# scrasmussen/uoparallel-seismic-project

Hardware: NVIDIA B200
Metric: GRelax/s (higher is better)
Workload: dtype f32

## Files before the change

include/sweeptt.h:

```cpp
#ifndef SWEEPTT_H
#define SWEEPTT_H

#include <stddef.h>
#include <stdint.h>

#ifdef __cplusplus
extern "C" {
#endif

#ifndef SWEEPTT_NO_STRUCTS
struct FS {
  int i, j, k;
  float d;
};

struct START {
  int i, j, k;
};
#endif

enum {
  SWEEPTT_KERNEL_AUTO = 0,
  SWEEPTT_KERNEL_SIMPLE = 1,
  SWEEPTT_KERNEL_TILED = 2
// ... 138 lines not shown
  int struct_size;
  double damp, smooth;
  double atol, btol, conlim;
  int iter_lim;
} sweeptt_lsqr_opts;

typedef struct {
  int struct_size;
  int istop, itn;
  double r1norm, r2norm, anorm, acond, arnorm, xnorm;
} sweeptt_lsqr_info;

int sweeptt_rayset_lsqr(sweeptt_rayset *set, const uint8_t *rows,
                        const double *b,
                        const sweeptt_lsqr_opts *opts,
                        double *x_out,
                        sweeptt_lsqr_info *info,
                        sweeptt_stats *stats);


enum { SWEEPTT_LOC_OK = 0, SWEEPTT_LOC_NO_PICKS = 1, SWEEPTT_LOC_UNREACHED = 2 };

int sweeptt_locate_events(sweeptt_ctx *ctx, int source_begin, int source_count, const float *picks, int nev,
                          struct START *best_out, float *misfit_out, double *origin_out,
                          int32_t *npicks_out, int32_t *status_out, sweeptt_stats *stats);

int sweeptt_misfit_box(sweeptt_ctx *ctx, int source_begin, int source_count, const float *picks ,
                       float *misfit_out, sweeptt_stats *stats);

long long sweeptt_relaxations_per_round(sweeptt_ctx *ctx);
size_t sweeptt_pool_bytes(sweeptt_ctx *ctx);
long long sweeptt_tiles_per_source(sweeptt_ctx *ctx);
int sweeptt_debug_model_stats(sweeptt_ctx *ctx, float *vmin, float *vmax, float *vpos);


int sweeptt_solve_slabs(const float *slowness, int nx, int ny, int nz, const struct FS *fs,
                        int starsize, struct START start, float *tt_out, const sweeptt_opts *opts,
                        sweeptt_stats *stats);

int sweeptt_solve_slabs_vbox(const char *vbox_path, const struct FS *fs, int starsize, struct START start,
                             float *tt_out, const sweeptt_opts *opts, sweeptt_stats *stats);


int sweeptt_vbox_load(const char *path, float **slowness, int origin[3], int dims[3]);
int sweeptt_vbox_dims(const char *path, int dims[3]);
int sweeptt_vbox_store(const char *path, const float *slowness, const int origin[3],
                       const int dims[3]);
int sweeptt_vbox_load_subset(const char *path, const int sub_origin[3], const int sub_dims[3],
                             float **slowness);
int sweeptt_text_load(const char *path, float **slowness, int origin[3], int dims[3]);
int sweeptt_star_load(const char *path, float delta, struct FS **fs, int *starsize);
int sweeptt_starts_load(const char *path, struct START **starts, int *numstart);
int sweeptt_write_output_tt(const char *path, const float *const *tt, int numstart, int nx, int ny,
                            int nz);
void sweeptt_free(void *p);

#ifdef __cplusplus
}
#endif
#endif
```

uoparallel_seismic_project_b200/api.py:

```python
from __future__ import annotations

import ctypes as C
import os
import pathlib
import weakref
from dataclasses import dataclass

import numpy as np

_PKG = pathlib.Path(__file__).resolve().parent
_LIB = None

KERNEL_AUTO, KERNEL_SIMPLE, KERNEL_TILED = 0, 1, 2
LOOP_AUTO, LOOP_BATCHED, LOOP_GRAPH = 0, 1, 2
RAY_OK, RAY_UNREACHED, RAY_NOT_FIXED_POINT, RAY_NO_PREDECESSOR, RAY_STALLED, RAY_TRUNCATED = range(6)
LOC_OK, LOC_NO_PICKS, LOC_UNREACHED = range(3)


class SweepError(RuntimeError):
    pass


class FS(C.Structure):
    _fields_ = [("i", C.c_int), ("j", C.c_int), ("k", C.c_int), ("d", C.c_float)]
# ... 42 lines not shown
    relaxations: int = 0
    solve_ms: float = 0.0
    relax_kernel_ms: float = 0.0
    relax_launches: int = 0
    h2d_ms: float = 0.0
    d2h_ms: float = 0.0
    h2d_bytes: int = 0
    d2h_bytes: int = 0
    units_run: int = 0
    units_changed: int = 0

    @classmethod
    def _from(cls, s: _Stats) -> "SweepStats":
        return cls(**{f: getattr(s, f) for f in cls.__dataclass_fields__})


def lib_path() -> pathlib.Path:
    import os
    if os.environ.get("SWEEPTT_LIB"):
        return pathlib.Path(os.environ["SWEEPTT_LIB"])
    return _PKG / "lib" / "libsweeptt.so"


_EXPORTS = [
    "sweeptt_device_count", "sweeptt_device_info", "sweeptt_last_error", "sweeptt_version",
    "sweeptt_star_fill_distances", "sweeptt_build_pull_star", "sweeptt_debug_column_split", "sweeptt_solve", "sweeptt_release_cache",
    "sweeptt_host_alloc", "sweeptt_host_free",
    "sweeptt_create", "sweeptt_destroy", "sweeptt_set_stream", "sweeptt_set_model", "sweeptt_set_star",
    "sweeptt_set_sources", "sweeptt_run", "sweeptt_step", "sweeptt_reset", "sweeptt_get_tt", "sweeptt_put_tt",
    "sweeptt_count_violations", "sweeptt_trace_rays", "sweeptt_ray_project", "sweeptt_ray_backproject",
    "sweeptt_rayset_freeze", "sweeptt_rayset_destroy", "sweeptt_rayset_bytes", "sweeptt_rayset_table",
    "sweeptt_rayset_paths", "sweeptt_rayset_project", "sweeptt_rayset_backproject", "sweeptt_rayset_lsqr",
    "sweeptt_locate_events",
    "sweeptt_misfit_box", "sweeptt_relaxations_per_round", "sweeptt_pool_bytes", "sweeptt_tiles_per_source", "sweeptt_debug_model_stats", "sweeptt_solve_slabs",
    "sweeptt_solve_slabs_vbox", "sweeptt_vbox_dims",
    "sweeptt_vbox_load", "sweeptt_vbox_store", "sweeptt_vbox_load_subset", "sweeptt_text_load",
    "sweeptt_star_load", "sweeptt_starts_load", "sweeptt_write_output_tt", "sweeptt_free",
]


def load_library() -> C.CDLL:
    global _LIB
    if _LIB is not None:
        return _LIB
    p = lib_path()
    if not p.exists():
        raise SweepError(f"{p} is missing: run `python -c 'import __graft_entry__ as g; g.build()'` "
                         "(the sweep has no CPU fallback)")
    lib = C.CDLL(str(p))
    fp, ip = C.POINTER(C.c_float), C.POINTER(C.c_int)
    lib.sweeptt_last_error.restype = C.c_char_p
    lib.sweeptt_version.restype = C.c_char_p
    lib.sweeptt_device_info.argtypes = [C.c_int, C.c_char_p, C.c_int, ip, ip, C.POINTER(C.c_size_t)]
    lib.sweeptt_star_fill_distances.argtypes = [C.POINTER(FS), C.c_int, C.c_float]
    lib.sweeptt_star_fill_distances.restype = None
    lib.sweeptt_build_pull_star.argtypes = [C.POINTER(FS), C.c_int, C.c_int, C.c_void_p, C.c_void_p, C.c_void_p, C.c_int]
    lib.sweeptt_solve.argtypes = [C.c_void_p, C.c_int, C.c_int, C.c_int, C.POINTER(FS), C.c_int, C.POINTER(START),
                                  C.c_int, C.POINTER(C.c_void_p), C.POINTER(_Opts), C.POINTER(_Stats)]
    lib.sweeptt_release_cache.restype = None
    lib.sweeptt_host_alloc.argtypes = [C.c_size_t]
    lib.sweeptt_host_alloc.restype = C.c_void_p
    lib.sweeptt_host_free.argtypes = [C.c_void_p]
    lib.sweeptt_host_free.restype = None
    lib.sweeptt_create.argtypes = [C.POINTER(_Opts)]
    lib.sweeptt_create.restype = C.c_void_p
    lib.sweeptt_destroy.argtypes = [C.c_void_p]
    lib.sweeptt_destroy.restype = None
# ... 7 lines not shown
    lib.sweeptt_get_tt.argtypes = [C.c_void_p, C.c_int, C.c_void_p]
    lib.sweeptt_put_tt.argtypes = [C.c_void_p, C.c_int, C.c_void_p]
    lib.sweeptt_count_violations.argtypes = [C.c_void_p, C.c_int, C.POINTER(C.c_longlong)]
    lib.sweeptt_trace_rays.argtypes = [C.c_void_p, C.c_int, C.c_int, C.POINTER(START), C.c_int, C.c_int, C.c_void_p,
                                       C.c_void_p, C.c_void_p, C.c_void_p, C.POINTER(_Stats)]
    lib.sweeptt_ray_project.argtypes = [C.c_void_p, C.c_int, C.c_int, C.POINTER(START), C.c_int, C.c_int, C.c_void_p,
                                        C.c_void_p, C.c_void_p, C.c_void_p, C.POINTER(_Stats)]
    lib.sweeptt_ray_backproject.argtypes = [C.c_void_p, C.c_int, C.c_int, C.POINTER(START), C.c_int, C.c_int,
                                            C.c_void_p, C.c_void_p, C.POINTER(C.c_int), C.c_void_p, C.POINTER(_Stats)]
    lib.sweeptt_rayset_freeze.argtypes = [C.c_void_p, C.c_int, C.c_int, C.POINTER(START), C.c_int, C.c_int,
                                          C.POINTER(_Stats)]
    lib.sweeptt_rayset_freeze.restype = C.c_void_p
    lib.sweeptt_rayset_destroy.argtypes = [C.c_void_p]
    lib.sweeptt_rayset_destroy.restype = None
    lib.sweeptt_rayset_bytes.argtypes = [C.c_void_p]
    lib.sweeptt_rayset_bytes.restype = C.c_size_t
    lib.sweeptt_rayset_table.argtypes = [C.c_void_p, C.c_void_p, C.c_void_p, C.c_void_p]
    lib.sweeptt_rayset_paths.argtypes = [C.c_void_p, C.c_void_p, C.c_void_p]
    lib.sweeptt_rayset_project.argtypes = [C.c_void_p, C.c_void_p, C.c_void_p, C.POINTER(_Stats)]
    lib.sweeptt_rayset_backproject.argtypes = [C.c_void_p, C.c_void_p, C.c_void_p, C.POINTER(C.c_int),
                                               C.POINTER(_Stats)]
    lib.sweeptt_rayset_lsqr.argtypes = [C.c_void_p, C.c_void_p, C.c_void_p, C.POINTER(_LsqrOpts), C.c_void_p,
                                        C.POINTER(_LsqrInfo), C.POINTER(_Stats)]
    lib.sweeptt_locate_events.argtypes = [C.c_void_p, C.c_int, C.c_int, C.c_void_p, C.c_int, C.c_void_p, C.c_void_p,
                                          C.c_void_p, C.c_void_p, C.c_void_p, C.POINTER(_Stats)]
    lib.sweeptt_misfit_box.argtypes = [C.c_void_p, C.c_int, C.c_int, C.c_void_p, C.c_void_p, C.POINTER(_Stats)]
    lib.sweeptt_relaxations_per_round.argtypes = [C.c_void_p]
    lib.sweeptt_relaxations_per_round.restype = C.c_longlong
    lib.sweeptt_pool_bytes.argtypes = [C.c_void_p]
    lib.sweeptt_pool_bytes.restype = C.c_size_t
    lib.sweeptt_tiles_per_source.argtypes = [C.c_void_p]
    lib.sweeptt_tiles_per_source.restype = C.c_longlong
    lib.sweeptt_debug_model_stats.argtypes = [C.c_void_p, C.c_void_p, C.c_void_p, C.c_void_p]
    lib.sweeptt_solve_slabs.argtypes = [C.c_void_p, C.c_int, C.c_int, C.c_int, C.POINTER(FS), C.c_int, START,
                                        C.c_void_p, C.POINTER(_Opts), C.POINTER(_Stats)]
    lib.sweeptt_solve_slabs_vbox.argtypes = [C.c_char_p, C.POINTER(FS), C.c_int, START, C.c_void_p, C.POINTER(_Opts),
                                             C.POINTER(_Stats)]
    lib.sweeptt_vbox_dims.argtypes = [C.c_char_p, ip]
    lib.sweeptt_vbox_load.argtypes = [C.c_char_p, C.POINTER(fp), ip, ip]
    lib.sweeptt_vbox_store.argtypes = [C.c_char_p, C.c_void_p, ip, ip]
    lib.sweeptt_vbox_load_subset.argtypes = [C.c_char_p, ip, ip, C.POINTER(fp)]
    lib.sweeptt_text_load.argtypes = [C.c_char_p, C.POINTER(fp), ip, ip]
    lib.sweeptt_star_load.argtypes = [C.c_char_p, C.c_float, C.POINTER(C.POINTER(FS)), ip]
    lib.sweeptt_starts_load.argtypes = [C.c_char_p, C.POINTER(C.POINTER(START)), ip]
    lib.sweeptt_write_output_tt.argtypes = [C.c_char_p, C.POINTER(C.c_void_p), C.c_int, C.c_int, C.c_int, C.c_int]
    lib.sweeptt_free.argtypes = [C.c_void_p]
    lib.sweeptt_free.restype = None
    _LIB = lib
    return lib


def _check(ok, what: str):
    if not ok:
        raise SweepError(f"{what}: {load_library().sweeptt_last_error().decode()}")


def device_count() -> int:
    return load_library().sweeptt_device_count()


def make_star(offsets, delta: float = 10.0):
    off = np.asarray(offsets, dtype=np.int32).reshape(-1, 3)
    arr = (FS * len(off))()
    for l, (a, b, c) in enumerate(off):
        arr[l].i, arr[l].j, arr[l].k = int(a), int(b), int(c)
    load_library().sweeptt_star_fill_distances(arr, len(off), C.c_float(delta))
# ... 376 lines not shown
                                               status.ctypes.data, C.byref(s)), "sweeptt_locate_events")
        return Locations(node, misfit, origin, npicks, status, SweepStats._from(s))

    def misfit_box(self, picks, sources=None) -> np.ndarray:
        begin, count = self._source_range(sources, "misfit_box")
        p = np.ascontiguousarray(picks, dtype=np.float32)
        if p.shape != (count,):
            raise SweepError(f"misfit_box: picks of shape {p.shape}, expected ({count},)")
        if self.dims is None:
            raise SweepError("misfit_box: the context needs a model first")
        out = np.empty(self.dims, np.float32)
        s = _Stats()
        _check(self._lib.sweeptt_misfit_box(self._h, begin, count, p.ctypes.data, out.ctypes.data, C.byref(s)),
               "sweeptt_misfit_box")
        return out

    @property
    def relaxations_per_round(self) -> int:
        return self._lib.sweeptt_relaxations_per_round(self._h)

    @property
    def tiles_per_source(self) -> int:
        return self._lib.sweeptt_tiles_per_source(self._h)

    @property
    def pool_bytes(self) -> int:
        return self._lib.sweeptt_pool_bytes(self._h)

    def model_stats(self):
        out = np.zeros(3, np.float32)
        _check(self._lib.sweeptt_debug_model_stats(self._h, out[0:].ctypes.data, out[1:].ctypes.data,
                                                   out[2:].ctypes.data), "sweeptt_debug_model_stats")
        return tuple(out)


class RaySet:

    def __init__(self, ctx: SweepContext, handle, shape, dims, stats: SweepStats):
        self._lib = ctx._lib
        self._ctx = ctx
        self._h = handle
        self.shape = shape
        self.dims = dims
        self.stats = stats
        self.length = np.empty(shape, np.int32)
        self.status = np.empty(shape, np.int32)
        self.tt = np.empty(shape, np.float32)
        _check(self._lib.sweeptt_rayset_table(self._h, self.length.ctypes.data, self.status.ctypes.data,
                                              self.tt.ctypes.data), "sweeptt_rayset_table")

    def _handle(self):
        if not self._h:
            raise SweepError("ray set is closed")
        return self._h

    def close(self):
        if getattr(self, "_h", None):
            self._lib.sweeptt_rayset_destroy(self._h)
            self._h = None

    __del__ = close

    def __enter__(self):
        return self

    def __exit__(self, *a):
# ... 210 lines not shown
```

uoparallel_seismic_project_b200/csrc/device_types.h:

```cpp
#pragma once
#include <cstdint>

namespace sweeptt {

#ifndef SWEEPTT_TX
#define SWEEPTT_TX 8
#endif
constexpr int TX = SWEEPTT_TX, TY = 8, TZ = 8, KZ = 8;
static_assert(TX == 4 || TX == 8, "a tile is one or two 4x8x8 units");
constexpr int UNITS = TX / 4;
constexpr int ZHALO = 8;
constexpr int SZD = TZ + 2 * ZHALO + 4;
constexpr int WIN = KZ + 2 * ZHALO;
#ifndef SWEEPTT_NW
#define SWEEPTT_NW 16
#endif
constexpr int MAX_WARPS = SWEEPTT_NW;
constexpr int XREACH = (7 + TX - 1) / TX;
constexpr int NMARK = (2 * XREACH + 1) * 9;

constexpr int AX = 7, AY = 7, AZ = ZHALO;

struct BoxGeom {
  int nx, ny, nz;
  int perm[3];
  long long dstride[3];
  int px, py, pz;
  int ntx, nty, ntz;
  long long sx;
  long long vol;
};

struct SolveState {
  int round;
  int last_changed_round;
  int parity;
  unsigned count[2];
  unsigned cursor;
  unsigned ticket;
  unsigned long long tile_visits;
  unsigned long long pulls;
  unsigned long long units_run;
  unsigned long long units_changed;
  int max_rounds;
  unsigned kmin_bits;
  unsigned ticket2;
  unsigned kmin_pub;
  unsigned gen;
  unsigned builder;
  unsigned done;
  unsigned inflight;
  unsigned long long gslot[4];
};

struct ColumnDev {
  int soff;
  unsigned kmask;
  int hd_begin;
  unsigned gmask;
};

struct ExtraDev {
  int i, j, k;
  int soff;
  float hd;
  int guarded;
  int pad0, pad1;
};

struct StarDev {
  int i, j, k;
  float hd;
  int guarded;
};

struct RayPull {
  short i, j, k;
  unsigned short rank;
  int off;
  float hd;
};
constexpr unsigned RAY_GUARD_BIT = 0x8000u;
constexpr int RAY_MAX_PULLS = 1 << 15;

constexpr int MAX_PARTS = 16;
// ... 9 lines not shown
```

uoparallel_seismic_project_b200/csrc/kernels.cu:

```cuda
#include "kernels.h"

#include "../../include/sweeptt.h"

#include <cuda_runtime.h>
#include <math_constants.h>

#include <algorithm>
#include <cstdint>
#include <limits>

#ifdef SWEEPTT_DEBUG_BOUNDS
#include <cstdio>
#define DBG_BOUNDS(cond)                                                                                        \
  do {                                                                                                          \
    if (!(cond)) {                                                                                              \
      printf("sweeptt bounds check failed: %s (kernels.cu:%d, block %d, thread %d)\n", #cond, __LINE__, (int)blockIdx.x, \
             (int)(threadIdx.y * blockDim.x + threadIdx.x));                                                    \
      __trap();                                                                                                 \
    }                                                                                                           \
  } while (0)
#else
#define DBG_BOUNDS(cond) do { } while (0)
#endif

// ... 353 lines not shown
    const unsigned thr = all ? 0x7f7fffffu : __float_as_uint(kmin + a.bucket);
    const float scale = a.bin_scale;
#pragma unroll 8
    for (unsigned i = tid; i < total; i += NCT) {
      const unsigned k = cache[i];
      if (k != 0x7f800000u && k <= thr) {
        const int b = min(GEN_BINS - 1, (int)((__uint_as_float(k) - kmin) * scale));
        atomicAdd(&s_bin[b + 1], 1u);
      }
    }
    __syncthreads();
    if (tid == 0)
      for (int b = 0; b < GEN_BINS; ++b) s_bin[b + 1] += s_bin[b];
    __syncthreads();
    const unsigned cnt = s_bin[GEN_BINS];
    __syncthreads();
#pragma unroll 8
    for (unsigned i = tid; i < total; i += NCT) {
      const unsigned k = cache[i];
      if (k != 0x7f800000u && k <= thr) {
        const int b = min(GEN_BINS - 1, (int)((__uint_as_float(k) - kmin) * scale));
        wl[atomicAdd(&s_bin[b], 1u)] = i;
        a.key[i] = 0x7f800000u;
        a.busy[i] = 1u;
      }
    }
    __threadfence();
    __syncthreads();
    if (tid == 0) {
      if (cnt != 0) {
        atomicAdd(&S->inflight, cnt);
        atomicExch(&S->gslot[g_new & 3u], (unsigned long long)cnt << 32);
        S->round += 1;
        __threadfence();
        st_volatile_u32(&S->gen, g_new);
        s_stop = 1u;
      } else if (early) {
        st_volatile_u32(&S->builder, g_new - 1u);
        s_stop = 1u;
      } else if (s_inflight == 0u) {
        st_volatile_u32(&S->done, 1u);
        s_stop = 1u;
      } else if (spins > (1u << 22)) {
        st_volatile_u32(&S->done, 2u);
        s_stop = 1u;
      } else {
        __nanosleep(200);
      }
    }
    __syncthreads();
    if (s_stop) break;
  }
}

template <int RXY, typename STAR, int NW, bool PERSIST>
__global__ void __block_size__((32, NW, 1))
relax_tiled(const __grid_constant__ CUtensorMap tm_slow, const __grid_constant__ CUtensorMap tm_tt,
            const __grid_constant__ RelaxArgs a) {
  using D = TileDims<RXY>;
  constexpr int NCT = 32 * NW;
  constexpr int FEED_TID = 32 * (NW / 2 - 1), FIN_WARP = NW - 1;
  extern __shared__ __align__(1024) unsigned char smem_raw[];
  float* ring = reinterpret_cast<float*>(smem_raw + ((128u - (smem_u32(smem_raw) & 127u)) & 127u));
  unsigned* s_acc = reinterpret_cast<unsigned*>(ring + 4 * D::BOX_STRIDE);
  __shared__ __align__(8) uint64_t full[2];
  __shared__ int s_tile[2];
  __shared__ unsigned s_gen;
  __shared__ int s_role;
  __shared__ unsigned s_tmin;
  __shared__ unsigned s_tmax;

  const int lane = threadIdx.x;
  const int wq = threadIdx.y;
  const int tid = wq * 32 + lane;
  if (tid == 0) {
    mbar_init(&full[0], 1); mbar_init(&full[1], 1);
    fence_mbar_init();
    s_tmin = 0x7f800000u;
    s_tmax = 0u;
    s_gen = 0u;
  }
  for (int i = tid; i < D::ACC_WORDS; i += NCT) s_acc[i] = 0x7f800000u;
  __syncthreads();

  SolveState* S = a.st;
  const int par = S->parity;
  const unsigned cnt = S->count[par];
  const unsigned* wl = a.worklist + (size_t)par * a.cap;
  const int round = S->round;
  const int ntiles = a.g.ntx * a.g.nty * a.g.ntz;

  auto stage_tile = [&](int q, int tile) {
    s_tile[q] = tile;
    if (tile < 0) {
      mbar_arrive(&full[q]);
      return;
    }
    if constexpr (PERSIST) fence_proxy_async_global();
    const int s = tile / ntiles;
    int tp = tile - s * ntiles;
    const int tz = tp % a.g.ntz; tp /= a.g.ntz;
    const int ty = tp % a.g.nty;
    const int tx = tp / a.g.nty;
    float* sv = ring + q * 2 * D::BOX_STRIDE;
    DBG_BOUNDS(tile >= 0 && s >= 0 && s < a.nsrc && tx >= 0 && tx < a.g.ntx);
    DBG_BOUNDS(tz * TZ + AZ - ZHALO >= 0 && tz * TZ + AZ - ZHALO + SZD <= a.g.pz);
    DBG_BOUNDS(ty * TY + AY - RXY >= 0 && ty * TY + AY - RXY + D::SYD <= a.g.py);
    DBG_BOUNDS(tx * TX + AX - RXY >= 0 && tx * TX + AX - RXY + D::SXD <= a.g.px);
    DBG_BOUNDS(a.slow_pb == 0 || (a.tx_owner[tx] == a.part && a.tx_slow0[tx] >= 0));
    mbar_expect_tx(&full[q], 2u * sizeof(float) * D::BOX_FLOATS);
    int cx = tx * TX + AX - RXY;
    if (a.slow_pb) cx = a.tx_slow0[tx] + (AX - RXY);
    tma_load_3d(sv, &tm_slow, &full[q], tz * TZ + AZ - ZHALO, ty * TY + AY - RXY, cx);
// ... 32 lines not shown
      const int dx = m / 9 - XREACH, dy = (m / 3) % 3 - 1, dz = m % 3 - 1;
      const int ux = wtx + dx, uy = wty + dy, uz = wtz + dz;
      const bool self = (dx == 0 && dy == 0 && dz == 0);
      bool reach = (abs(dx) - 1) * TX < RXY;
      if (self && !wself) reach = false;
      if (reach && ux >= 0 && ux < a.g.ntx && uy >= 0 && uy < a.g.nty && uz >= 0 && uz < a.g.ntz) {
        const size_t u = (size_t)ws * ntiles + ((size_t)ux * a.g.nty + uy) * a.g.ntz + uz;
        unsigned* keyp = a.key;
        const unsigned* tmaxp = a.tmax;
        if constexpr (!PERSIST) {
          if (a.nparts > 1) {
            const int o = a.tx_owner[ux];
            if ((which == 1 && o != a.part) || (which == 2 && o == a.part)) continue;
            keyp = a.part_key[o];
            tmaxp = a.part_tmax[o];
          }
        }
        bool useful = true;
        if (tmaxp != nullptr && !self)
          useful = __float_as_uint(__fadd_rn(__uint_as_float(wtmin), a.dmin)) < __ldcg(&tmaxp[u]);
        if (useful) atomicMin(&keyp[u], wtmin);
      }
    }
  };
  for (uint32_t it = 0;; ++it) {
    const int q = it & 1;
    mbar_wait(&full[q], (it >> 1) & 1);
    const int tile = s_tile[q];
    if (tile == TILE_NONE) break;
    if constexpr (PERSIST) {
      if (tile == TILE_NEXT_GEN || tile == TILE_BUILD) {
        const bool early = tile == TILE_BUILD;
        __syncthreads();
        for (;;) {
          if (tid == 0) {
            const unsigned g = s_gen;
            int role = 0;
            if (ld_volatile_u32(&S->done)) role = 0;
            else if (ld_volatile_u32(&S->gen) != g) role = 0;
            else if (atomicCAS(&S->builder, g, g + 1u) == g) role = 2;
            else role = early ? 0 : 1;
            s_role = role;
          }
          __syncthreads();
          const int role = s_role;
          __syncthreads();
          if (role == 2) {
          const size_t nkeys = (size_t)a.nsrc * ntiles;
          build_generation<NCT>(a, s_gen + 1u,
                                nkeys <= (size_t)4 * D::BOX_STRIDE ? reinterpret_cast<unsigned*>(ring) : a.keysnap, early);
            fence_proxy_async_all();
            __syncthreads();
            break;
          }
          if (role == 0) break;
          if (tid == 0) {
            unsigned spins = 0;
            while (ld_volatile_u32(&S->gen) == s_gen && !ld_volatile_u32(&S->done) &&
                   ld_volatile_u32(&S->builder) != s_gen) {
              __nanosleep(100);
              if (++spins > (1u << 24)) { st_volatile_u32(&S->done, 2u); break; }
            }
          }
          __syncthreads();
        }
        if (tid == 0) stage_tile(q ^ 1, pop_now());
        continue;
      }
    }
    unsigned pop_i = 0, pop_g = 0, pop_c = 0;
    unsigned long long pop_w = 0;
    int next_tile = TILE_NONE;
    const bool build_now = build_next;
    build_next = false;
    if (tid == FEED_TID) {
      if constexpr (PERSIST) pop_g = s_gen;
      else pop_i = atomicAdd(&S->cursor, 1u);
    }
    const int s = tile / ntiles;
    int tp = tile - s * ntiles;
    const int tz = tp % a.g.ntz; tp /= a.g.ntz;
    const int ty = tp % a.g.nty;
    const int tx = tp / a.g.nty;
    const int x0 = tx * TX, y0 = ty * TY, z0 = tz * TZ;
    const float* sv = ring + q * 2 * D::BOX_STRIDE;
    float* st = ring + q * 2 * D::BOX_STRIDE + D::BOX_STRIDE;

    const int nlive = (UNITS == 2 && x0 + 4 < a.g.nx) ? 2 : 1;
    const int P = NW / nlive;
    const int unit = wq / P, part = wq - unit * P;
    const int xc = tx == 0 ? 1 : (tx == a.g.ntx - 1 ? 2 : 0);
    int f0 = ((xc * 6 + ((PERSIST || a.nparts > 1) ? 3 : 0) + (nlive == 1 ? 0 : 1 + unit)) * MAX_PATTERNS) * MAX_WARPS + part;
#ifndef SWEEPTT_NO_PIN
    asm volatile("" : "+r"(f0));
#endif
    const bool owner = part == 0;
    const int x = (unit << 2) | (lane >> 3);
    const int b0 = ((x + RXY) * D::SYD + (y + RXY)) * SZD;
// ... 1233 lines not shown
    default: return cudaErrorInvalidValue;
  }
  return cudaGetLastError();
}
cudaError_t launch_relax_tiled(const TiledLaunch& tl, const CUtensorMap& tm_slow, const CUtensorMap& tm_tt,
                               const RelaxArgs& a, cudaStream_t stream) {
  return launch_relax_any(tl, tm_slow, tm_tt, a, false, stream);
}
cudaError_t launch_relax_persistent(const TiledLaunch& tl, const CUtensorMap& tm_slow, const CUtensorMap& tm_tt,
                                    const RelaxArgs& a, cudaStream_t stream) {
  return launch_relax_any(tl, tm_slow, tm_tt, a, true, stream);
}
cudaError_t launch_persist_check(const RelaxArgs& a, cudaStream_t stream) {
  const size_t total = (size_t)a.nsrc * a.g.ntx * a.g.nty * a.g.ntz;
  scan_min_key<<<(unsigned)std::min<size_t>(296, (total + 255) / 256), 256, 0, stream>>>(a);
  return cudaGetLastError();
}
size_t tiled_persistent_max_keys(int rxy) {
  switch (rxy) {
    case 2: return 4 * (size_t)TileDims<2>::BOX_STRIDE;
    case 4: return 4 * (size_t)TileDims<4>::BOX_STRIDE;
    case 7: return 4 * (size_t)TileDims<7>::BOX_STRIDE;
  }
  return 0;
}
__global__ void persist_begin_kernel(const RelaxArgs a) {
  SolveState* S = a.st;
  const unsigned cnt = S->count[0];
  for (unsigned i = threadIdx.x; i < cnt; i += blockDim.x) a.busy[a.worklist[i]] = 1u;
  if (threadIdx.x == 0) {
    S->gen = 0u; S->builder = 0u; S->done = 0u;
    S->inflight = cnt;
    S->gslot[0] = (unsigned long long)cnt << 32;
  }
}
cudaError_t launch_persist_begin(const RelaxArgs& a, cudaStream_t stream) {
  const size_t total = (size_t)a.nsrc * a.g.ntx * a.g.nty * a.g.ntz;
  cudaError_t e = cudaMemsetAsync(a.busy, 0, total * sizeof(unsigned), stream);
  if (e != cudaSuccess) return e;
  persist_begin_kernel<<<1, 256, 0, stream>>>(a);
  return cudaGetLastError();
}

constexpr int FUSED_MAX_KEYS = 49152;
constexpr int FUSED_BINS = 32;
__global__ void __launch_bounds__(1024) compact_fused(const RelaxArgs a, unsigned long long cond) {
  extern __shared__ unsigned s_keys[];
  __shared__ unsigned s_min;
  __shared__ unsigned s_bin[FUSED_BINS + 1];
  SolveState* S = a.st;
  const int nxt = S->parity ^ 1;
  const unsigned total = (unsigned)((size_t)a.nsrc * a.g.ntx * a.g.nty * a.g.ntz);
  if (threadIdx.x == 0) s_min = 0x7f800000u;
  if (threadIdx.x <= FUSED_BINS) s_bin[threadIdx.x] = 0;
  __syncthreads();
  unsigned m = 0x7f800000u;
#pragma unroll 8
  for (unsigned i = threadIdx.x; i < total; i += 1024) {
    const unsigned k = a.key[i];
    s_keys[i] = k;
    m = min(m, k);
  }
  m = __reduce_min_sync(0xffffffffu, m);
  if ((threadIdx.x & 31) == 0 && m != 0x7f800000u) atomicMin(&s_min, m);
  __syncthreads();
  if (a.nparts > 1) {
// ... 349 lines not shown
```

uoparallel_seismic_project_b200/csrc/kernels.h:

```cpp
#pragma once
#include <cuda.h>
#include <cuda_runtime.h>

#include "device_types.h"

namespace sweeptt {

struct TiledLaunch {
  int rxy;
  int stock_id;
  int nw;
  int grid;
  int grid_persistent;
  size_t smem_bytes;
};

int tiled_variant_for_radius(int r);
void tiled_variant_dims(int rxy, int* sxd, int* syd, int* szd);
cudaError_t tiled_prepare(int rxy, int stock_id, int device, TiledLaunch* out);
int tiled_stock_star_for(const uint32_t* masks_ascending, int n, int rxy_needed);

cudaError_t upload_star_constants(const ColumnDev* cols, int ncols, const float* col_hd, int nhd,
                                  const ExtraDev* extra, int nextra, const unsigned* pdesc, int npdesc,
                                  cudaStream_t stream);

struct RelaxArgs {
  BoxGeom g;
  const float* slow;
  float* tt;
  int nsrc;
  const int* src_xyz;
  SolveState* st;
  unsigned* worklist;
  unsigned cap;
  unsigned* key;
  unsigned* tmax;
  float dmin;
  unsigned* busy;
  unsigned* keysnap;
  float bin_scale;
  float bucket;
  const unsigned long long* tile_pulls;
  int ncols, nextra;
  int max_inner;
  float neg_zero;
  unsigned lookahead;
  unsigned trig_q8;
  int nparts;
  int part;
  const unsigned char* tx_owner;
  const int* tx_slow0;
  int slow_pb;
  unsigned* part_key[MAX_PARTS];
  unsigned* part_tmax[MAX_PARTS];
  unsigned* part_kmin[MAX_PARTS];
  float front_slack;
  int npat;
  int pat_begin[MAX_PATTERNS + 1];
};

cudaError_t launch_relax_tiled(const TiledLaunch& tl, const CUtensorMap& tm_slow,
                               const CUtensorMap& tm_tt, const RelaxArgs& a, cudaStream_t stream);
cudaError_t launch_relax_persistent(const TiledLaunch& tl, const CUtensorMap& tm_slow, const CUtensorMap& tm_tt,
                                    const RelaxArgs& a, cudaStream_t stream);
cudaError_t launch_persist_begin(const RelaxArgs& a, cudaStream_t stream);
cudaError_t launch_persist_check(const RelaxArgs& a, cudaStream_t stream);
size_t tiled_persistent_max_keys(int rxy);
cudaError_t launch_compact(const RelaxArgs& a, unsigned long long cond, cudaStream_t stream);

cudaError_t launch_relax_simple(const RelaxArgs& a, const StarDev* star, int nstar,
                                unsigned long long pulls_per_round, cudaStream_t stream);
cudaError_t launch_advance_simple(SolveState* st, unsigned long long cond, cudaStream_t stream);

cudaError_t launch_reset_part(const RelaxArgs& a, int max_rounds, cudaStream_t stream);
cudaError_t launch_init_sources(const RelaxArgs& a, cudaStream_t stream);

cudaError_t launch_count_violations(const RelaxArgs& a, int source, const StarDev* star, int nstar,
                                    unsigned long long* out, cudaStream_t stream);

struct TraceArgs {
// ... 105 lines not shown
```

uoparallel_seismic_project_b200/csrc/solver.cu:

```cuda
#include <cuda.h>
#include <cudaTypedefs.h>
#include <cuda_runtime.h>

#include <algorithm>
#include <array>
#include <atomic>
#include <chrono>
#include <condition_variable>
#include <cmath>
#include <cstdarg>
#include <cstdio>
#include <cstdlib>
#include <cstring>
#include <functional>
#include <limits>
#include <map>
#include <mutex>
#include <string>
#include <thread>
#include <tuple>
#include <vector>

#include "../../include/sweeptt.h"
#include "kernels.h"
// ... 139 lines not shown
  size_t loc_cap = 0;
  size_t pool_bytes = 0;

  std::vector<FS> fs;
  PullStar star;
  StarDev* d_star = nullptr;
  int nstar = 0;
  long long pulls_per_round = 0;

  int kernel_used = 0;
  TiledLaunch tl{};
  CUtensorMap tm_slow{}, tm_tt{};
  bool maps_valid = false;
  int consts_rxy = -1;
  std::vector<ColumnDev> img_cols;
  std::vector<float> img_hd;
  std::vector<ExtraDev> img_extra;
  std::vector<unsigned> img_pdesc;
  int consts_nx = -1;
  uint64_t img_sig = 0;
  std::vector<int> pat_begin;
  std::vector<unsigned short> psplit;
  std::vector<PullColumn> dev_columns;

  cudaGraphExec_t graph_exec = nullptr;
  bool graph_valid = false;

  struct Slice {
    int wave = 0;
    int s0 = 0, ns = 0;
    int slot = 1;
    int lane = 0;
    bool persistent = false;
    int grid = 0;
    cudaGraphExec_t graph = nullptr;
    CUtensorMap tm_tt{};
  };
  std::vector<Slice> plan;
  int plan_waves = 0;
  bool plan_valid = false;
  std::vector<cudaStream_t> aux_streams;
  std::vector<cudaEvent_t> aux_done;
  cudaEvent_t ev_fork = nullptr;

  cudaStream_t copy_stream = nullptr;
  float* d_out_ring = nullptr;
  float* h_out_ring = nullptr;
  size_t out_ring_boxes = 0, out_ring_box_floats = 0;
  std::vector<cudaEvent_t> ring_unpadded, ring_copied;

  std::vector<cudaEvent_t> prof_events;
  bool allow_outside_sources = false;
  int max_inner = 1;
  int force_window_axis = -1;
  int force_x_axis = -1;
  bool external_boxes = false;
  int slow_pb = 0;
  long long slow_planes = 0;
  int mp_nparts = 0, mp_part = 0;
  unsigned char* d_tx_owner = nullptr;
  int* d_tx_slow0 = nullptr;
  unsigned* mp_key[MAX_PARTS] = {};
  unsigned* mp_tmax[MAX_PARTS] = {};
  unsigned* mp_kmin[MAX_PARTS] = {};
};

namespace {
struct ConstTables {
  std::mutex mu;
  std::condition_variable cv;
  uint64_t sig = 0;
  bool loaded = false;
// ... 803 lines not shown
}

static int persistent_capacity(sweeptt_ctx* c) {
  if (c->kernel_used != SWEEPTT_KERNEL_TILED || c->opts.max_rounds > 0) return 0;
  if (c->tl.nw < MAX_WARPS && !getenv("SWEEPTT_PERSIST")) return 0;
  if (const char* e = getenv("SWEEPTT_PERSIST")) { if (atoi(e) == 0) return 0; }
  if (env_loop(c) == SWEEPTT_LOOP_BATCHED) return 0;
  size_t max_keys = tiled_persistent_max_keys(c->tl.rxy);
  if (const char* e = getenv("SWEEPTT_PERSIST_MAX_KEYS")) max_keys = (size_t)atoll(e);
  const size_t ntiles = (size_t)c->g.ntx * c->g.nty * c->g.ntz;
  return (int)std::min<size_t>(max_keys / ntiles, 1u << 20);
}

static int build_plan(sweeptt_ctx* c) {
  if (c->plan_valid) return 1;
  invalidate_graph(c);
  const int cap = persistent_capacity(c);
  int wave_size = 0;
  bool persistent = false;
  if (cap >= 1) {
    const int nwaves = (c->nsrc + cap - 1) / cap;
    wave_size = (c->nsrc + nwaves - 1) / nwaves;
    persistent = true;
  }
  if (const char* e = getenv("SWEEPTT_WAVE")) {
    const int w = atoi(e);
    if (w <= 0) { wave_size = c->nsrc; persistent = cap >= c->nsrc; }
    else { wave_size = std::min(w, c->nsrc); persistent = cap >= wave_size; }
  }
  if (wave_size <= 0) wave_size = c->nsrc;
  int want_groups = 2;
  if (const char* env = getenv("SWEEPTT_GROUPS")) want_groups = atoi(env);
  want_groups = std::max(1, std::min(want_groups, MAX_GROUPS));
  int kstreams = 1;
  if (const char* e = getenv("SWEEPTT_WAVE_STREAMS")) kstreams = std::max(1, std::min(atoi(e), MAX_GROUPS));
  const int nwaves_total = (c->nsrc + wave_size - 1) / wave_size;
  if (!persistent || nwaves_total < 2 * kstreams) kstreams = 1;
  if (c->opts.profile_kernels) kstreams = 1;
  std::vector<int> sizes;
  if (persistent && c->nsrc > wave_size && c->nsrc >= 8 && !getenv("SWEEPTT_WAVE")) {
    const int last = std::min(4, wave_size);
    const int rest = c->nsrc - last;
    const int nw = (rest + wave_size - 1) / wave_size;
    for (int w = 0; w < nw; ++w) sizes.push_back((int)((long long)rest * (w + 1) / nw - (long long)rest * w / nw));
    sizes.push_back(last);
  } else {
    for (int s0 = 0; s0 < c->nsrc; s0 += wave_size) sizes.push_back(std::min(wave_size, c->nsrc - s0));
  }
  int slot = 1, wave = 0;
  for (int s0 = 0; wave < (int)sizes.size(); s0 += sizes[wave], ++wave) {
    const int ns = sizes[wave];
    const int parts = persistent ? 1 : std::min(want_groups, ns);
    for (int g = 0; g < parts; ++g) {
      sweeptt_ctx::Slice sl;
      sl.wave = persistent ? wave / kstreams : wave;
      sl.s0 = s0 + (int)((long long)ns * g / parts);
      sl.ns = s0 + (int)((long long)ns * (g + 1) / parts) - sl.s0;
      sl.slot = slot++;
      sl.lane = persistent ? wave % kstreams : g;
      sl.grid = (persistent && kstreams > 1) ? std::max(1, c->tl.grid_persistent / kstreams) : 0;
      sl.persistent = persistent;
      if (slot > STATE_SLOTS) return fail("too many slices in the solve plan (%d sources in waves of %d)", c->nsrc, wave_size);
      c->plan.push_back(sl);
    }
  }
  c->plan_waves = persistent ? (wave + kstreams - 1) / kstreams : wave;
  int lanes = 1;
  for (const auto& sl : c->plan) lanes = std::max(lanes, sl.lane + 1);
  while ((int)c->aux_streams.size() < lanes - 1) {
    cudaStream_t st;
    cudaEvent_t ev;
    CK(cudaStreamCreateWithFlags(&st, cudaStreamNonBlocking));
    CK(cudaEventCreateWithFlags(&ev, cudaEventDisableTiming));
    c->aux_streams.push_back(st);
    c->aux_done.push_back(ev);
  }
  for (auto& sl : c->plan) {
    if (c->kernel_used == SWEEPTT_KERNEL_TILED && !encode_tt_map(c, c->d_tt + (size_t)sl.s0 * c->g.vol, sl.ns, &sl.tm_tt)) return 0;
    if (!sl.persistent) {
      cudaStream_t st = sl.lane ? c->aux_streams[sl.lane - 1] : c->stream;
      if (!build_while_graph(c, slice_args(c, sl), sl.tm_tt, st, &sl.graph)) return 0;
    }
  }
  c->plan_valid = true;
  return 1;
}

static void fill_stats(sweeptt_ctx* c, sweeptt_stats* st, int rounds_before, long long launches, long long relax_launches,
                       double relax_ms) {
  if (!st) return;
  const SolveState& h = *c->h_state;
  st->struct_size = sizeof(sweeptt_stats);
  st->rounds = h.round - rounds_before;
  st->kernel_used = c->kernel_used;
  st->devices_used = 1;
  st->kernel_launches = launches;
  st->relax_launches = relax_launches;
  st->tile_visits = (long long)h.tile_visits;
  st->relaxations = (long long)h.pulls;
// ... 69 lines not shown
                                                                  : (h.last_changed_round < h.round);
      if (done) break;
      if (c->opts.max_rounds > 0 && h.round - rounds_before >= c->opts.max_rounds) break;
      if (c->opts.verbose > 0)
        fprintf(stderr, "[sweeptt] round %d: %u tiles queued, %llu pulls so far\n", h.round, h.count[h.parity], h.pulls);
    }
  }
  if (changed_out)
    *changed_out = (c->kernel_used == SWEEPTT_KERNEL_TILED) ? (c->h_state->count[c->h_state->parity] != 0)
                                                            : (c->h_state->last_changed_round == c->h_state->round);
  fill_stats(c, stats, rounds_before, launches, relax_launches, relax_ms);
  return 1;
}

static int run_plan(sweeptt_ctx* c, sweeptt_stats* stats, const std::function<int(int, int, cudaStream_t)>& after_wave) {
  if (!build_plan(c)) return 0;
  const bool profile = c->opts.profile_kernels != 0;
  size_t ev_used = 0;
  CK(cudaEventRecord(c->ev0, c->stream));
  CK(cudaEventRecord(c->ev_fork, c->stream));
  std::vector<char> lane_used(1 + c->aux_streams.size(), 0);
  auto lane_stream = [&](int lane) -> cudaStream_t {
    cudaStream_t st = lane ? c->aux_streams[lane - 1] : c->stream;
    if (lane && !lane_used[lane]) cudaStreamWaitEvent(st, c->ev_fork, 0);
    lane_used[lane] = 1;
    return st;
  };
  size_t i = 0;
  while (i < c->plan.size()) {
    if (c->plan[i].persistent) {
      const auto& sl = c->plan[i];
      cudaStream_t st = lane_stream(sl.lane);
      RelaxArgs a = slice_args(c, sl);
      TiledLaunch tl = c->tl;
      if (sl.ns < 6 && !getenv("SWEEPTT_LOOKAHEAD")) a.lookahead /= 2;
      if (sl.grid > 0) {
        a.lookahead = (unsigned)((unsigned long long)a.lookahead * sl.grid / std::max(1, tl.grid_persistent));
        tl.grid_persistent = sl.grid;
      }
      CK(launch_reset(a, c->opts.max_rounds, st));
      CK(launch_persist_begin(a, st));
      if (profile) {
        while (c->prof_events.size() < ev_used + 2) {
          cudaEvent_t e;
          CK(cudaEventCreate(&e));
          c->prof_events.push_back(e);
        }
        CK(cudaEventRecord(c->prof_events[ev_used], st));
      }
      CK(launch_relax_persistent(tl, c->tm_slow, sl.tm_tt, a, st));
      if (profile) { CK(cudaEventRecord(c->prof_events[ev_used + 1], st)); ev_used += 2; }
      CK(launch_persist_check(a, st));
      if (after_wave && !after_wave(sl.s0, sl.ns, st)) return 0;
      ++i;
      continue;
    }
    const int wave = c->plan[i].wave;
    size_t j = i;
    while (j < c->plan.size() && c->plan[j].wave == wave) ++j;
    if (i > 0) {
      CK(cudaEventRecord(c->ev_fork, c->stream));
      for (size_t k = i; k < j; ++k)
        if (c->plan[k].lane) CK(cudaStreamWaitEvent(c->aux_streams[c->plan[k].lane - 1], c->ev_fork, 0));
    }
    for (size_t k = i; k < j; ++k) {
      const auto& sl = c->plan[k];
      cudaStream_t st = lane_stream(sl.lane);
      CK(launch_reset(slice_args(c, sl), c->opts.max_rounds, st));
      CK(cudaGraphLaunch(sl.graph, st));
      if (sl.lane) CK(cudaEventRecord(c->aux_done[sl.lane - 1], st));
    }
    for (size_t k = i; k < j; ++k)
      if (c->plan[k].lane) CK(cudaStreamWaitEvent(c->stream, c->aux_done[c->plan[k].lane - 1], 0));
    if (after_wave) {
      const int s0 = c->plan[i].s0, s1 = c->plan[j - 1].s0 + c->plan[j - 1].ns;
      if (!after_wave(s0, s1 - s0, c->stream)) return 0;
    }
    i = j;
  }
  for (size_t lane = 1; lane < lane_used.size(); ++lane)
    if (lane_used[lane] && !c->plan.empty() && c->plan[0].persistent) {
      CK(cudaEventRecord(c->aux_done[lane - 1], c->aux_streams[lane - 1]));
      CK(cudaStreamWaitEvent(c->stream, c->aux_done[lane - 1], 0));
    }
  CK(cudaEventRecord(c->ev1, c->stream));
  const size_t nslots = 1 + c->plan.size();
  CK(cudaMemcpyAsync(c->h_state, c->d_state, sizeof(SolveState) * nslots, cudaMemcpyDeviceToHost, c->stream));
  CK(launch_reset_state_only(c->d_state, c->opts.max_rounds, c->stream));
  CK(cudaStreamSynchronize(c->stream));
  float ms = 0;
  CK(cudaEventElapsedTime(&ms, c->ev0, c->ev1));
  if (stats) {
    std::memset(stats, 0, sizeof *stats);
    stats->struct_size = sizeof *stats;
    stats->kernel_used = c->kernel_used;
    stats->devices_used = 1;
    stats->solve_ms = ms;
    for (size_t e = 0; e < ev_used; e += 2) {
      float k = 0;
      CK(cudaEventElapsedTime(&k, c->prof_events[e], c->prof_events[e + 1]));
      stats->relax_kernel_ms += k;
    }
  }
  int pending = 0;
  for (const auto& sl : c->plan) {
    const SolveState& h = c->h_state[sl.slot];
    if (sl.persistent) {
      if (h.done != 1u || h.inflight != 0u || h.kmin_bits != 0x7f800000u)
        return fail("single-launch solve of sources %d..%d stopped without reaching the fixed point (done %u, in flight %u, "
                    "pending key %08x)", sl.s0, sl.s0 + sl.ns - 1, h.done, h.inflight, h.kmin_bits);
    } else {
      pending |= (c->kernel_used == SWEEPTT_KERNEL_TILED) ? (h.count[h.parity] != 0) : (h.last_changed_round == h.round);
    }
    if (stats) {
      const long long per_reset = (c->kernel_used == SWEEPTT_KERNEL_TILED && make_args(c).tmax) ? 5 : 4;
      stats->rounds = std::max(stats->rounds, h.round);
      if (sl.persistent) {
        stats->kernel_launches += per_reset + 3;
        stats->relax_launches += 1;
      } else {
        stats->kernel_launches += (c->kernel_used == SWEEPTT_KERNEL_TILED ? 3LL : 2LL) * h.round + per_reset;
        stats->relax_launches += h.round;
      }
      stats->tile_visits += (long long)h.tile_visits;
      stats->relaxations += (long long)h.pulls;
      stats->units_run += (long long)h.units_run;
      stats->units_changed += (long long)h.units_changed;
    }
  }
  if (pending && c->opts.max_rounds > 0) return fail("not converged after max_rounds = %d rounds", c->opts.max_rounds);
  return 1;
}

static bool plan_usable(sweeptt_ctx* c) {
  const int loop = env_loop(c);
  if (loop == SWEEPTT_LOOP_BATCHED) return false;
  if (c->opts.profile_kernels) {
    const int cap = persistent_capacity(c);
    if (cap < 1) return false;
    if (const char* e = getenv("SWEEPTT_WAVE")) { const int w = atoi(e); if (w <= 0 ? cap < c->nsrc : cap < std::min(w, c->nsrc)) return false; }
    return true;
  }
  return true;
}

static int run_locked(sweeptt_ctx* c, sweeptt_stats* stats, const std::function<int(int, int, cudaStream_t)>& after_wave) {
  if (stats) { std::memset(stats, 0, sizeof *stats); }
  if (plan_usable(c)) return run_plan(c, stats, after_wave);
  CK(cudaEventRecord(c->ev0, c->stream));
  CK(launch_reset(make_args(c), c->opts.max_rounds, c->stream));
  int changed = 0;
  if (!run_rounds(c, true, 0, &changed, stats)) return 0;
  CK(cudaEventRecord(c->ev1, c->stream));
  CK(cudaEventSynchronize(c->ev1));
  float ms = 0;
  CK(cudaEventElapsedTime(&ms, c->ev0, c->ev1));
  if (stats) { stats->solve_ms = ms; stats->kernel_launches += 4; }
  if (changed && c->opts.max_rounds > 0) return fail("not converged after max_rounds = %d rounds", c->opts.max_rounds);
  if (after_wave && !after_wave(0, c->nsrc, c->stream)) return 0;
  return 1;
}

extern "C" int sweeptt_run(sweeptt_ctx* c, sweeptt_stats* stats) {
  ConstLease lease;
  if (!ready(c, &lease)) return 0;
  return run_locked(c, stats, nullptr);
}

extern "C" int sweeptt_step(sweeptt_ctx* c, int rounds, int* changed, sweeptt_stats* stats) {
  ConstLease lease;
  if (!ready(c, &lease)) return 0;
  if (rounds < 1) return fail("sweeptt_step: rounds must be >= 1");
  if (stats) std::memset(stats, 0, sizeof *stats);
  CK(cudaEventRecord(c->ev0, c->stream));
  if (!run_rounds(c, false, rounds, changed, stats)) return 0;
  CK(cudaEventRecord(c->ev1, c->stream));
  CK(cudaEventSynchronize(c->ev1));
  float ms = 0;
  CK(cudaEventElapsedTime(&ms, c->ev0, c->ev1));
  if (stats) stats->solve_ms = ms;
// ... 1111 lines not shown
  if (!picks || !misfit_out) return fail("%s: picks and misfit_out are required", who);
  ConstLease lease;
  LocateArgs a;
  if (!locate_prepare(c, &lease, who, source_begin, source_count, picks, 1, &a, nullptr, stats)) return 0;
  const size_t dense = (size_t)c->g.nx * c->g.ny * c->g.nz;
  if (!ensure_stage(c, dense)) return 0;
  CK(cudaEventRecord(c->ev0, c->stream));
  CK(launch_misfit_box(a, c->d_stage, c->stream));
  CK(cudaEventRecord(c->ev1, c->stream));
  CK(cudaEventSynchronize(c->ev1));
  float ms = 0;
  CK(cudaEventElapsedTime(&ms, c->ev0, c->ev1));
  const auto t_copy = std::chrono::steady_clock::now();
  CK(cudaMemcpyAsync(misfit_out, c->d_stage, dense * 4, cudaMemcpyDeviceToHost, c->stream));
  CK(cudaStreamSynchronize(c->stream));
  if (stats) {
    stats->solve_ms = ms;
    stats->kernel_launches = 1;
    stats->d2h_ms = std::chrono::duration<double, std::milli>(std::chrono::steady_clock::now() - t_copy).count();
    stats->d2h_bytes = (long long)dense * 4;
  }
  return 1;
}

extern "C" long long sweeptt_relaxations_per_round(sweeptt_ctx* c) { return c ? c->pulls_per_round : 0; }
extern "C" size_t sweeptt_pool_bytes(sweeptt_ctx* c) { return c ? c->pool_bytes : 0; }
extern "C" int sweeptt_debug_model_stats(sweeptt_ctx* c, float* vmin, float* vmax, float* vpos) {
  if (!c || !c->have_model) return fail("sweeptt_debug_model_stats: no model");
  if (vmin) *vmin = c->min_slowness;
  if (vmax) *vmax = c->max_slowness;
  if (vpos) *vpos = c->pos_slowness;
  return 1;
}
extern "C" long long sweeptt_tiles_per_source(sweeptt_ctx* c) {
  return (c && c->have_model) ? (long long)c->g.ntx * c->g.nty * c->g.ntz : 0;
}

static std::mutex g_cache_mu;
namespace { struct CacheEntry; }
extern "C" void sweeptt_release_cache(void);

namespace {
struct CacheEntry {
  std::mutex busy;
  sweeptt_ctx* ctx = nullptr;
};
std::map<int, CacheEntry*> g_cache_entries;
struct CachedCtx {
  CacheEntry* e = nullptr;
  sweeptt_ctx* ctx = nullptr;
  CachedCtx(int device, const sweeptt_opts& o) {
    {
      std::lock_guard<std::mutex> lk(g_cache_mu);
      auto it = g_cache_entries.find(device);
      if (it == g_cache_entries.end()) it = g_cache_entries.emplace(device, new CacheEntry()).first;
      e = it->second;
    }
    e->busy.lock();
    if (e->ctx) {
      sweeptt_ctx* c = e->ctx;
      const bool star_opts_changed = c->opts.star_used != o.star_used || c->opts.kernel != o.kernel;
      const bool plan_opts_changed = c->opts.loop != o.loop || c->opts.max_rounds != o.max_rounds ||
                                     c->opts.profile_kernels != o.profile_kernels;
      c->opts = o;
      c->opts.device = device;
      if (star_opts_changed) c->have_star = false;
// ... 685 lines not shown
```

Baseline: 5182.

## Let persistent wave blocks exit early so the next wave's kernel can start

```diff
diff --git a/include/sweeptt.h b/include/sweeptt.h
--- a/include/sweeptt.h
+++ b/include/sweeptt.h
@@ -194,6 +194,7 @@
 size_t sweeptt_pool_bytes(sweeptt_ctx *ctx);
 long long sweeptt_tiles_per_source(sweeptt_ctx *ctx);
 int sweeptt_debug_model_stats(sweeptt_ctx *ctx, float *vmin, float *vmax, float *vpos);
+long long sweeptt_debug_wave_exits(sweeptt_ctx *ctx);
 
 
 int sweeptt_solve_slabs(const float *slowness, int nx, int ny, int nz, const struct FS *fs,
diff --git a/uoparallel_seismic_project_b200/api.py b/uoparallel_seismic_project_b200/api.py
--- a/uoparallel_seismic_project_b200/api.py
+++ b/uoparallel_seismic_project_b200/api.py
@@ -98,7 +98,8 @@
     "sweeptt_rayset_freeze", "sweeptt_rayset_destroy", "sweeptt_rayset_bytes", "sweeptt_rayset_table",
     "sweeptt_rayset_paths", "sweeptt_rayset_project", "sweeptt_rayset_backproject", "sweeptt_rayset_lsqr",
     "sweeptt_locate_events",
-    "sweeptt_misfit_box", "sweeptt_relaxations_per_round", "sweeptt_pool_bytes", "sweeptt_tiles_per_source", "sweeptt_debug_model_stats", "sweeptt_solve_slabs",
+    "sweeptt_misfit_box", "sweeptt_relaxations_per_round", "sweeptt_pool_bytes", "sweeptt_tiles_per_source", "sweeptt_debug_model_stats", "sweeptt_debug_wave_exits",
+    "sweeptt_solve_slabs",
     "sweeptt_solve_slabs_vbox", "sweeptt_vbox_dims",
     "sweeptt_vbox_load", "sweeptt_vbox_store", "sweeptt_vbox_load_subset", "sweeptt_text_load",
     "sweeptt_star_load", "sweeptt_starts_load", "sweeptt_write_output_tt", "sweeptt_free",
@@ -172,6 +173,8 @@
     lib.sweeptt_tiles_per_source.argtypes = [C.c_void_p]
     lib.sweeptt_tiles_per_source.restype = C.c_longlong
     lib.sweeptt_debug_model_stats.argtypes = [C.c_void_p, C.c_void_p, C.c_void_p, C.c_void_p]
+    lib.sweeptt_debug_wave_exits.argtypes = [C.c_void_p]
+    lib.sweeptt_debug_wave_exits.restype = C.c_longlong
     lib.sweeptt_solve_slabs.argtypes = [C.c_void_p, C.c_int, C.c_int, C.c_int, C.POINTER(FS), C.c_int, START,
                                         C.c_void_p, C.POINTER(_Opts), C.POINTER(_Stats)]
     lib.sweeptt_solve_slabs_vbox.argtypes = [C.c_char_p, C.POINTER(FS), C.c_int, START, C.c_void_p, C.POINTER(_Opts),
@@ -614,6 +617,9 @@
         _check(self._lib.sweeptt_debug_model_stats(self._h, out[0:].ctypes.data, out[1:].ctypes.data,
                                                    out[2:].ctypes.data), "sweeptt_debug_model_stats")
         return tuple(out)
+
+    def wave_exits(self) -> int:
+        return self._lib.sweeptt_debug_wave_exits(self._h)
 
 
 class RaySet:
diff --git a/uoparallel_seismic_project_b200/csrc/device_types.h b/uoparallel_seismic_project_b200/csrc/device_types.h
--- a/uoparallel_seismic_project_b200/csrc/device_types.h
+++ b/uoparallel_seismic_project_b200/csrc/device_types.h
@@ -51,6 +51,10 @@
   unsigned done;
   unsigned inflight;
   unsigned long long gslot[4];
+  unsigned active;
+  unsigned gen_size;
+  unsigned gen_peak;
+  unsigned left;
 };
 
 struct ColumnDev {
diff --git a/uoparallel_seismic_project_b200/csrc/kernels.cu b/uoparallel_seismic_project_b200/csrc/kernels.cu
--- a/uoparallel_seismic_project_b200/csrc/kernels.cu
+++ b/uoparallel_seismic_project_b200/csrc/kernels.cu
@@ -409,6 +409,8 @@
         atomicAdd(&S->inflight, cnt);
         atomicExch(&S->gslot[g_new & 3u], (unsigned long long)cnt << 32);
         S->round += 1;
+        st_volatile_u32(&S->gen_size, cnt);
+        if (cnt > ld_volatile_u32(&S->gen_peak)) st_volatile_u32(&S->gen_peak, cnt);
         __threadfence();
         st_volatile_u32(&S->gen, g_new);
         s_stop = 1u;
@@ -428,6 +430,21 @@
     __syncthreads();
     if (s_stop) break;
   }
+}
+
+__device__ __forceinline__ bool leave_wave(SolveState* S) {
+  const unsigned size = ld_volatile_u32(&S->gen_size);
+  unsigned n = ld_volatile_u32(&S->active);
+  if (size >= ld_volatile_u32(&S->gen_peak) || size >= n) return false;
+  while (n > 1u) {
+    const unsigned was = atomicCAS(&S->active, n, n - 1u);
+    if (was == n) {
+      atomicAdd(&S->left, 1u);
+      return true;
+    }
+    n = was;
+  }
+  return false;
 }
 
 template <int RXY, typename STAR, int NW, bool PERSIST>
@@ -456,6 +473,11 @@
     s_tmin = 0x7f800000u;
     s_tmax = 0u;
     s_gen = 0u;
+    if constexpr (PERSIST) {
+      atomicAdd(&a.st->active, 1u);
+      const unsigned g = ld_volatile_u32(&a.st->gen);
+      s_gen = g > 0u ? g - 1u : 0u;
+    }
   }
   for (int i = tid; i < D::ACC_WORDS; i += NCT) s_acc[i] = 0x7f800000u;
   __syncthreads();
@@ -554,12 +576,14 @@
       if (tile == TILE_NEXT_GEN || tile == TILE_BUILD) {
         const bool early = tile == TILE_BUILD;
         __syncthreads();
+        bool leave = false;
         for (;;) {
           if (tid == 0) {
             const unsigned g = s_gen;
             int role = 0;
             if (ld_volatile_u32(&S->done)) role = 0;
             else if (ld_volatile_u32(&S->gen) != g) role = 0;
+            else if (!early && a.may_leave && leave_wave(S)) role = 3;
             else if (atomicCAS(&S->builder, g, g + 1u) == g) role = 2;
             else role = early ? 0 : 1;
             s_role = role;
@@ -567,6 +591,7 @@
           __syncthreads();
           const int role = s_role;
           __syncthreads();
+          if (role == 3) { leave = true; break; }
           if (role == 2) {
           const size_t nkeys = (size_t)a.nsrc * ntiles;
           build_generation<NCT>(a, s_gen + 1u,
@@ -586,6 +611,7 @@
           }
           __syncthreads();
         }
+        if (leave) break;
         if (tid == 0) stage_tile(q ^ 1, pop_now());
         continue;
       }
@@ -1885,6 +1911,8 @@
     S->gen = 0u; S->builder = 0u; S->done = 0u;
     S->inflight = cnt;
     S->gslot[0] = (unsigned long long)cnt << 32;
+    S->active = 0u; S->left = 0u;
+    S->gen_size = cnt; S->gen_peak = cnt;
   }
 }
 cudaError_t launch_persist_begin(const RelaxArgs& a, cudaStream_t stream) {
diff --git a/uoparallel_seismic_project_b200/csrc/kernels.h b/uoparallel_seismic_project_b200/csrc/kernels.h
--- a/uoparallel_seismic_project_b200/csrc/kernels.h
+++ b/uoparallel_seismic_project_b200/csrc/kernels.h
@@ -46,6 +46,7 @@
   float neg_zero;
   unsigned lookahead;
   unsigned trig_q8;
+  int may_leave;
   int nparts;
   int part;
   const unsigned char* tx_owner;
diff --git a/uoparallel_seismic_project_b200/csrc/solver.cu b/uoparallel_seismic_project_b200/csrc/solver.cu
--- a/uoparallel_seismic_project_b200/csrc/solver.cu
+++ b/uoparallel_seismic_project_b200/csrc/solver.cu
@@ -195,12 +195,12 @@
     int slot = 1;
     int lane = 0;
     bool persistent = false;
-    int grid = 0;
     cudaGraphExec_t graph = nullptr;
     CUtensorMap tm_tt{};
   };
   std::vector<Slice> plan;
   int plan_waves = 0;
+  long long wave_exits = 0;
   bool plan_valid = false;
   std::vector<cudaStream_t> aux_streams;
   std::vector<cudaEvent_t> aux_done;
@@ -1070,11 +1070,7 @@
   int want_groups = 2;
   if (const char* env = getenv("SWEEPTT_GROUPS")) want_groups = atoi(env);
   want_groups = std::max(1, std::min(want_groups, MAX_GROUPS));
-  int kstreams = 1;
-  if (const char* e = getenv("SWEEPTT_WAVE_STREAMS")) kstreams = std::max(1, std::min(atoi(e), MAX_GROUPS));
-  const int nwaves_total = (c->nsrc + wave_size - 1) / wave_size;
-  if (!persistent || nwaves_total < 2 * kstreams) kstreams = 1;
-  if (c->opts.profile_kernels) kstreams = 1;
+  const int kstreams = (persistent && !c->opts.profile_kernels) ? 2 : 1;
   std::vector<int> sizes;
   if (persistent && c->nsrc > wave_size && c->nsrc >= 8 && !getenv("SWEEPTT_WAVE")) {
     const int last = std::min(4, wave_size);
@@ -1091,18 +1087,17 @@
     const int parts = persistent ? 1 : std::min(want_groups, ns);
     for (int g = 0; g < parts; ++g) {
       sweeptt_ctx::Slice sl;
-      sl.wave = persistent ? wave / kstreams : wave;
+      sl.wave = wave;
       sl.s0 = s0 + (int)((long long)ns * g / parts);
       sl.ns = s0 + (int)((long long)ns * (g + 1) / parts) - sl.s0;
       sl.slot = slot++;
       sl.lane = persistent ? wave % kstreams : g;
-      sl.grid = (persistent && kstreams > 1) ? std::max(1, c->tl.grid_persistent / kstreams) : 0;
       sl.persistent = persistent;
       if (slot > STATE_SLOTS) return fail("too many slices in the solve plan (%d sources in waves of %d)", c->nsrc, wave_size);
       c->plan.push_back(sl);
     }
   }
-  c->plan_waves = persistent ? (wave + kstreams - 1) / kstreams : wave;
+  c->plan_waves = wave;
   int lanes = 1;
   for (const auto& sl : c->plan) lanes = std::max(lanes, sl.lane + 1);
   while ((int)c->aux_streams.size() < lanes - 1) {
@@ -1238,12 +1233,9 @@
       const auto& sl = c->plan[i];
       cudaStream_t st = lane_stream(sl.lane);
       RelaxArgs a = slice_args(c, sl);
-      TiledLaunch tl = c->tl;
+      const TiledLaunch& tl = c->tl;
       if (sl.ns < 6 && !getenv("SWEEPTT_LOOKAHEAD")) a.lookahead /= 2;
-      if (sl.grid > 0) {
-        a.lookahead = (unsigned)((unsigned long long)a.lookahead * sl.grid / std::max(1, tl.grid_persistent));
-        tl.grid_persistent = sl.grid;
-      }
+      a.may_leave = !profile && i + 1 < c->plan.size();
       CK(launch_reset(a, c->opts.max_rounds, st));
       CK(launch_persist_begin(a, st));
       if (profile) {
@@ -1309,9 +1301,11 @@
     }
   }
   int pending = 0;
+  c->wave_exits = 0;
   for (const auto& sl : c->plan) {
     const SolveState& h = c->h_state[sl.slot];
     if (sl.persistent) {
+      c->wave_exits += h.left;
       if (h.done != 1u || h.inflight != 0u || h.kmin_bits != 0x7f800000u)
         return fail("single-launch solve of sources %d..%d stopped without reaching the fixed point (done %u, in flight %u, "
                     "pending key %08x)", sl.s0, sl.s0 + sl.ns - 1, h.done, h.inflight, h.kmin_bits);
@@ -1352,6 +1346,7 @@
 
 static int run_locked(sweeptt_ctx* c, sweeptt_stats* stats, const std::function<int(int, int, cudaStream_t)>& after_wave) {
   if (stats) { std::memset(stats, 0, sizeof *stats); }
+  c->wave_exits = 0;
   if (plan_usable(c)) return run_plan(c, stats, after_wave);
   CK(cudaEventRecord(c->ev0, c->stream));
   CK(launch_reset(make_args(c), c->opts.max_rounds, c->stream));
@@ -2529,6 +2524,7 @@
   if (vpos) *vpos = c->pos_slowness;
   return 1;
 }
+extern "C" long long sweeptt_debug_wave_exits(sweeptt_ctx* c) { return c ? c->wave_exits : 0; }
 extern "C" long long sweeptt_tiles_per_source(sweeptt_ctx* c) {
   return (c && c->have_model) ? (long long)c->g.ntx * c->g.nty * c->g.ntz : 0;
 }
```

Result: faster. 5270 (median of 6 runs) (+1.7%).
